# kant2002/GGMLSharp

Hardware: AMD Instinct MI355X
Metric: effective GFLOP/s, Q4_0 mul_mat 4096x4096x4096 (2*M*K*N / step time) (higher is better)
Workload: dtype i8

## Files before the change

### ggmlsharp_amd/csrc/gemm_qmx.hip

```cpp
#include "common.h"
#include "plan.h"
#include <cstdlib>
#include <utility>

#if !defined(GGML_HIP_DEV)
#undef GGML_MX_DBG
#undef GGML_MX_XCD1D
#endif
#ifndef GGML_MX_DBG
#define GGML_MX_DBG 0
#endif
#ifndef GGML_MX_XCD1D
#define GGML_MX_XCD1D 0
#endif

namespace {

using f32x4 = __attribute__((ext_vector_type(4))) float;
using f32x16 = __attribute__((ext_vector_type(16))) float;
using u32x4 = __attribute__((ext_vector_type(4))) uint32_t;
using u32x2 = __attribute__((ext_vector_type(2))) uint32_t;
using i32x8 = __attribute__((ext_vector_type(8))) int;

typedef __attribute__((address_space(3))) void lds_void;
// ... 6 lines not shown
    __builtin_amdgcn_raw_ptr_buffer_load_lds(r, (lds_void *)l, 16, (int)voff, (int)soff, 0, 0);
}

template <typename F, int... Is>
__device__ __forceinline__ void static_for_impl(F &&f, std::integer_sequence<int, Is...>) {
    (f(std::integral_constant<int, Is>{}), ...);
}
template <int N, typename F>
__device__ __forceinline__ void static_for(F &&f) {
    static_for_impl(f, std::make_integer_sequence<int, N>{});
}

#ifdef K3M_CLOCK
__device__ unsigned long long k3m_clock_buf[8192 * 2];
__device__ unsigned int k3m_where_buf[8192 * 2];
#endif

#ifndef GGML_MX_FULLDRAIN
#define GGML_MX_FULLDRAIN 0
#endif
template <int TYPE, int WMT, int WNT, int WGM, int WGN, int KB>
struct Cfg {
    static constexpr int TM = WGM * WMT * 32, TN = WGN * WNT * 32, NT = WGM * WGN * 64;
    static constexpr int A16_BYTES = KB * 2 * TN * 16;
    static constexpr int A8_BYTES = KB * 2 * TN * 8;
    static constexpr int NSC = (TYPE == GGML_TYPE_Q4_1) ? 2 : 1;
    static constexpr int SC_BYTES = KB * TN * 4;
    static constexpr int STAGE = A16_BYTES + A8_BYTES + NSC * SC_BYTES;
    static constexpr int TOTAL = 2 * STAGE;
    static constexpr int P = NT / TN;
    static_assert(NT % TN == 0 && (P == 1 || P == 2 || P == 4), "chunk decomposition");
    static_assert((KB * 2 * TN) % NT == 0 && (KB * TN) % NT == 0, "DMA rounds");
    static constexpr int A16_ROUNDS = KB * 2 * TN / NT, A8_ROUNDS = KB * TN / NT;
    static constexpr int SC_CHUNKS = KB * TN / 4;
    static_assert((SC_CHUNKS % 64 == 0 || SC_CHUNKS == 32) && SC_CHUNKS <= NT, "scale DMA is whole waves (or the first half of one: 32-column tiles)");
    static constexpr int NPIECE = A16_ROUNDS + A8_ROUNDS + 1;
    static constexpr int DRAIN_T = (KB - 1) * WMT * WNT + WMT * WNT / 2;
    static constexpr int PP = (NPIECE + DRAIN_T - 1) / DRAIN_T;
    static_assert(PP <= 3, "at most three DMA pieces per tile");
};

template <int TYPE, int WMT, int WNT, int WGM, int WGN, int KB, int FB, int KSP, int VS>
__global__ __launch_bounds__(WGM * WGN * 64 * KSP, (VS > 1 && WGM * WGN * KSP == 4 && WMT * WNT == 2 ? 3 : 2))
void gemm_qmx_kernel(const uint8_t *__restrict__ w6a, const uint8_t *__restrict__ w6b, const float *__restrict__ wd,
                     const float *__restrict__ wm, const uint8_t *__restrict__ a6, const float *__restrict__ ad,
                     const float *__restrict__ asd, float *__restrict__ dst, int M, int N, int Mpad, int Npad, int nstages,
                     int ldd, int tiles_m, int tiles_n, uint32_t w6a_bytes, uint32_t wd_bytes, uint32_t a_bytes,
                     uint32_t ad_bytes, uint32_t dst_bytes, const mm_epilogue ep) {
    using C = Cfg<TYPE, WMT, WNT, WGM, WGN, KB>;
    constexpr int NTILE = WMT * WNT, P = C::P;
    constexpr int NF = (TYPE == GGML_TYPE_Q4_0 || TYPE == GGML_TYPE_Q4_1) ? 1 : 2;
    static_assert(KB % 2 == 0, "fragment buffers alternate by k-block parity");
    static_assert(VS == 1 || (KSP == 1 && (VS == 2 || VS == 4)) || (KSP == 2 && VS == 2), "virtual split forms");
    constexpr int KV = KSP * VS;
    extern __shared__ __attribute__((aligned(16))) uint8_t smem[];

    const int lane = threadIdx.x & 63;
    const int wave_all = __builtin_amdgcn_readfirstlane(threadIdx.x >> 6);
    const int grp = wave_all / (WGM * WGN);
    const int wave = wave_all % (WGM * WGN);
    const int tid = wave * 64 + lane;
    const int l31 = lane & 31, hh = lane >> 5;
    const int wn = wave / WGM, wm_ = wave % WGM;
    uint8_t *const gsm = smem + grp * C::TOTAL;

    const int nwg = tiles_m * tiles_n;
    const int bid = blockIdx.x, xcd = bid & 7, q8 = nwg >> 3, r8 = nwg & 7;
    int tm_i, tn_i;
// ... 144 lines not shown
                else asm volatile("s_waitcnt vmcnt(0)" ::: "memory");
            }
            if constexpr (t < LAST) issue(std::integral_constant<int, t + 1>{});
            f32x16 &ac = acc[i][j];
            static_for<4>([&](auto gc) {
                constexpr int q = decltype(gc)::value;
                float t0, t1, t2, t3;
                if constexpr (t == 0 && q == 0) asm volatile("s_nop 11" : "+v"(tacc[0]));
                if constexpr (q == 0 && t < LAST && TYPE == GGML_TYPE_Q4_1 && (((t + 1) / NTILE) & 1)) {
                    constexpr int tn = t + 1, j1 = (tn % NTILE) / WMT, i1 = tn % WMT;
                    asm volatile("" : "+v"(acc[i1][j1]));
                }
                if constexpr ((GGML_MX_DBG & 16) != 0) {
                    asm volatile("" : "+v"(ac[4 * q]) : "v"(tacc[t & 1]), "v"(da[q]), "v"(dw), "v"(tacc[(t + 1) & 1]));
                } else if constexpr (q == 0 && t < LAST) {
                    asm volatile("v_mul_f32 %4, %8, %12\n\tv_mul_f32 %5, %9, %13\n\tv_mul_f32 %6, %10, %14\n\tv_mul_f32 %7, %11, %15\n\t"
                                 "v_fmac_f32 %0, %4, %16\n\tv_fmac_f32 %1, %5, %16\n\tv_fmac_f32 %2, %6, %16\n\tv_fmac_f32 %3, %7, %16"
                                 : "+v"(ac[0]), "+v"(ac[1]), "+v"(ac[2]), "+v"(ac[3]), "=&v"(t0), "=&v"(t1), "=&v"(t2), "=&v"(t3)
                                 : "v"(tacc[t & 1][0]), "v"(tacc[t & 1][1]), "v"(tacc[t & 1][2]), "v"(tacc[t & 1][3]), "v"(da[0][0]),
                                   "v"(da[0][1]), "v"(da[0][2]), "v"(da[0][3]), "v"(dw), "v"(tacc[(t + 1) & 1]));
                } else {
                    asm volatile("v_mul_f32 %4, %8, %12\n\tv_mul_f32 %5, %9, %13\n\tv_mul_f32 %6, %10, %14\n\tv_mul_f32 %7, %11, %15\n\t"
                                 "v_fmac_f32 %0, %4, %16\n\tv_fmac_f32 %1, %5, %16\n\tv_fmac_f32 %2, %6, %16\n\tv_fmac_f32 %3, %7, %16"
                                 : "+v"(ac[4 * q + 0]), "+v"(ac[4 * q + 1]), "+v"(ac[4 * q + 2]), "+v"(ac[4 * q + 3]), "=&v"(t0), "=&v"(t1),
                                   "=&v"(t2), "=&v"(t3)
                                 : "v"(tacc[t & 1][4 * q + 0]), "v"(tacc[t & 1][4 * q + 1]), "v"(tacc[t & 1][4 * q + 2]),
                                   "v"(tacc[t & 1][4 * q + 3]), "v"(da[q][0]), "v"(da[q][1]), "v"(da[q][2]), "v"(da[q][3]), "v"(dw));
                }
                if constexpr (i == WMT - 1 && bb * WNT + j + 1 < KB * WNT && !(GGML_MX_DBG & (2 | 32)))
                    fetch_da(std::integral_constant<int, bb * WNT + j + 1>{}, gc);
            });
        });
    };

    static_assert(FB <= KB, "fragment look-ahead stays within two stages");
    const int s_first = grp * VS;
    static_for<C::NPIECE>([&](auto pc) { dma_piece(s_first, 0, pc); });
    static_for<WMT>([&](auto ic) {
// ... 2 lines not shown
    asm volatile("s_waitcnt vmcnt(0) lgkmcnt(0)" ::: "memory");
    __builtin_amdgcn_s_barrier();
    asm volatile("" ::: "memory");
    f32x16 sav[VS > 1 ? WMT : 1][VS > 1 ? WNT : 1];
    const int niter = VS * ((nstages + KV - 1) / KV);
    int sc = s_first, pass = 0;
#ifdef K3M_CLOCK
    const unsigned long long clk_c0 = __builtin_readcyclecounter(), clk_r0 = wall_clock64();
#endif
#ifndef GGML_MX_PRIO
#define GGML_MX_PRIO 15
#endif
#ifndef GGML_MX_PRIO_ON
#define GGML_MX_PRIO_ON 8
#endif
    bool younger = false;
    if constexpr (WGM * WGN * KSP == 4 && GGML_MX_PRIO != 0) {
        uint32_t hwid;
        asm volatile("s_getreg_b32 %0, hwreg(HW_REG_HW_ID)" : "=s"(hwid));
        younger = (hwid & 1u) != 0 && nwg <= 512;
    }
    for (int it = 0; it < niter; ++it) {
        if constexpr (WGM * WGN * KSP == 4 && GGML_MX_PRIO != 0) {
            if (younger) { if (it % GGML_MX_PRIO < GGML_MX_PRIO_ON) __builtin_amdgcn_s_setprio(1); else __builtin_amdgcn_s_setprio(0); }
        }
        int sn = sc + KV, pn = pass;
        if (VS > 1 && sn >= nstages) { pn = pass + 1; sn = pn < VS ? grp * VS + pn : nstages; }
        if ((KSP == 1 && VS == 1) || sc < nstages) compute(sc, sn, it);
        if constexpr (KSP == 1 && VS == 1 && !GGML_MX_FULLDRAIN) asm volatile("s_waitcnt lgkmcnt(0)" ::: "memory");
        else asm volatile("s_waitcnt vmcnt(0) lgkmcnt(0)" ::: "memory");
        if (!(GGML_MX_DBG & 1)) __builtin_amdgcn_s_barrier();
        asm volatile("" ::: "memory");
        if constexpr (VS > 1) {
            if (pn != pass && pn < VS) {
#pragma unroll
                for (int i = 0; i < WMT; ++i)
#pragma unroll
                    for (int j = 0; j < WNT; ++j) {
                        sav[i][j] = pass == 0 ? acc[i][j] : sav[i][j] + acc[i][j];
#pragma unroll
                        for (int r = 0; r < 16; ++r) acc[i][j][r] = 0.0f;
                    }
            }
        }
        sc = sn; pass = pn;
    }
#ifdef K3M_CLOCK
    {
        asm volatile("" : "+v"(acc[0][0]));
        const unsigned long long c1 = __builtin_readcyclecounter(), r1 = wall_clock64();
        const size_t slot = (size_t)blockIdx.x * (WGM * WGN * KSP) + wave_all;
        if (lane == 0 && slot < 8192) { k3m_clock_buf[2 * slot] = c1 - clk_c0; k3m_clock_buf[2 * slot + 1] = r1 - clk_r0; }
        uint32_t hw, xcc;
        asm volatile("s_getreg_b32 %0, hwreg(HW_REG_HW_ID)\n\ts_getreg_b32 %1, hwreg(HW_REG_XCC_ID)" : "=s"(hw), "=s"(xcc));
        if (lane == 0 && slot < 8192) { k3m_where_buf[2 * slot] = hw; k3m_where_buf[2 * slot + 1] = xcc; }
    }
#endif

    if constexpr (KSP > 1) {
        constexpr int GRP_FLOATS = WGM * WGN * NTILE * 16 * 64;
        static_assert((KSP - 1) * VS * GRP_FLOATS * 4 <= KSP * C::TOTAL, "K-split exchange fits the stage buffers");
        float *xch = (float *)smem + (size_t)wave * (NTILE * 16 * 64) + lane;
        if (grp != 0) {
#pragma unroll
            for (int i = 0; i < WMT; ++i)
#pragma unroll
                for (int j = 0; j < WNT; ++j)
#pragma unroll
                    for (int r = 0; r < 16; ++r) {
                        if constexpr (VS > 1) xch[(size_t)((grp - 1) * VS) * GRP_FLOATS + ((i * WNT + j) * 16 + r) * 64] = sav[i][j][r];
                        xch[(size_t)((grp - 1) * VS + VS - 1) * GRP_FLOATS + ((i * WNT + j) * 16 + r) * 64] = acc[i][j][r];
// ... 13 lines not shown
        const float *xch = (const float *)smem + (size_t)wave * (NTILE * 16 * 64) + lane;
#pragma unroll
        for (int g = VS; g < KV; ++g)
#pragma unroll
            for (int i = 0; i < WMT; ++i)
#pragma unroll
                for (int j = 0; j < WNT; ++j)
#pragma unroll
                    for (int r = 0; r < 16; ++r) acc[i][j][r] += xch[(size_t)(g - VS) * GRP_FLOATS + ((i * WNT + j) * 16 + r) * 64];
    }

    (void)dst_bytes;
    const rsrc_t rD = make_rsrc(dst + (size_t)n0 * ldd + m0, 0xFFFFFFFFu);
    const bool full = n0 + C::TN <= N && m0 + C::TM <= M;
    const uint32_t lane_off = (uint32_t)((4 * hh * ldd + l31) * 4);
    if (ep.mode == 3) {
        rsrc_t rP[MM_PUSH_MAX];
#pragma unroll
        for (int k = 0; k < MM_PUSH_MAX; ++k) rP[k] = make_rsrc((k < ep.npush ? ep.push[k] : dst) + (size_t)n0 * ldd + m0, 0xFFFFFFFFu);
#pragma unroll
        for (int i = 0; i < WMT; ++i)
#pragma unroll
            for (int j = 0; j < WNT; ++j) {
                const int mb = (wm_ * WMT + i) * 32, nb = (wn * WNT + j) * 32;
                if (m0 + mb >= M || n0 + nb >= N) continue;
                const bool mok = m0 + mb + l31 < M;
#pragma unroll
                for (int r = 0; r < 16; ++r) {
                    const int nr = nb + (r & 3) + 8 * (r >> 2);
                    const float v = acc[i][j][r];
                    if (!(mok && n0 + nr + 4 * hh < N)) continue;
                    const uint32_t so = (uint32_t)(nr * ldd + mb) * 4u, vb = __builtin_bit_cast(uint32_t, v);
                    __builtin_amdgcn_raw_buffer_store_b32(vb, rD, (int)lane_off, (int)so, 0);
#pragma unroll
                    for (int k = 0; k < MM_PUSH_MAX; ++k)
                        if (k < ep.npush) __builtin_amdgcn_raw_buffer_store_b32(vb, rP[k], (int)lane_off, (int)so, 0);
                }
            }
        return;
    }
    if (ep.mode != 0) {
        const int lda = (int)ep.ld_add, ld2 = (int)ep.ld2;
        const rsrc_t rS = make_rsrc(ep.mode == 1 ? ep.addend + (size_t)n0 * lda + m0 : dst, 0xFFFFFFFFu);
        const rsrc_t rD2 = make_rsrc(ep.mode == 1 ? ep.dst2 + (size_t)n0 * ld2 + m0 : dst, 0xFFFFFFFFu);
        const uint32_t lane_s = (uint32_t)((4 * hh * lda + l31) * 4), lane_2 = (uint32_t)((4 * hh * ld2 + l31) * 4);
#pragma unroll
        for (int i = 0; i < WMT; ++i)
#pragma unroll
            for (int j = 0; j < WNT; ++j) {
                const int mb = (wm_ * WMT + i) * 32, nb = (wn * WNT + j) * 32;
                if (m0 + mb >= M || n0 + nb >= N) continue;
                const bool mok = m0 + mb + l31 < M;
#pragma unroll
                for (int r = 0; r < 16; ++r) {
                    const int nr = nb + (r & 3) + 8 * (r >> 2);
                    const float v = acc[i][j][r];
                    if (!(mok && n0 + nr + 4 * hh < N)) continue;
                    if (ep.mode == 2) {
                        const float o = v * ep.scale;
                        __builtin_amdgcn_raw_buffer_store_b32(__builtin_bit_cast(uint32_t, o), rD, (int)lane_off, (int)((uint32_t)(nr * ldd + mb) * 4u), 0);
                    } else {
                        __builtin_amdgcn_raw_buffer_store_b32(__builtin_bit_cast(uint32_t, v), rD, (int)lane_off, (int)((uint32_t)(nr * ldd + mb) * 4u), 0);
                        const float a = __builtin_bit_cast(float, __builtin_amdgcn_raw_buffer_load_b32(rS, (int)lane_s, (int)((uint32_t)(nr * lda + mb) * 4u), 0));
                        const float o = v + a;
                        __builtin_amdgcn_raw_buffer_store_b32(__builtin_bit_cast(uint32_t, o), rD2, (int)lane_2, (int)((uint32_t)(nr * ld2 + mb) * 4u), 0);
                    }
                }
            }
        return;
    }
    if (full) {
#pragma unroll
        for (int i = 0; i < WMT; ++i)
#pragma unroll
            for (int j = 0; j < WNT; ++j)
#pragma unroll
                for (int r = 0; r < 16; ++r) {
                    const int nr = (wn * WNT + j) * 32 + (r & 3) + 8 * (r >> 2), mb = (wm_ * WMT + i) * 32;
                    const float v = acc[i][j][r];
                    __builtin_amdgcn_raw_buffer_store_b32(__builtin_bit_cast(uint32_t, v), rD, (int)lane_off,
                                                          (int)((uint32_t)(nr * ldd + mb) * 4u), 0);
                }
    } else {
#pragma unroll
        for (int i = 0; i < WMT; ++i)
#pragma unroll
            for (int j = 0; j < WNT; ++j) {
                const int mb = (wm_ * WMT + i) * 32, nb = (wn * WNT + j) * 32;
                if (m0 + mb >= M || n0 + nb >= N) continue;
                const bool mok = m0 + mb + l31 < M;
#pragma unroll
                for (int r = 0; r < 16; ++r) {
                    const int nr = nb + (r & 3) + 8 * (r >> 2);
                    const float v = acc[i][j][r];
                    if (mok && n0 + nr + 4 * hh < N)
                        __builtin_amdgcn_raw_buffer_store_b32(__builtin_bit_cast(uint32_t, v), rD, (int)lane_off,
                                                              (int)((uint32_t)(nr * ldd + mb) * 4u), 0);
                }
            }
    }
}

#ifdef K3S_TRACE
__device__ unsigned long long k3s_trace_buf[2048 * 2 * 8];
#define K3S_STAMP(k) do { if (lane == 0 && (wave == 0 || wave == KS - 1) && blockIdx.x < 2048) \
        k3s_trace_buf[((size_t)blockIdx.x * 2 + (wave != 0)) * 8 + (k)] = wall_clock64(); } while (0)
#else
#define K3S_STAMP(k) do { } while (0)
#endif
template <int TYPE, int KS, int NP, bool ROT, int WMT>
__device__ __forceinline__
void gemm_qmx_small_body(const uint8_t *__restrict__ w6a, const uint8_t *__restrict__ w6b, const float *__restrict__ wd,
                         const float *__restrict__ wm, const uint8_t *__restrict__ a6, const float *__restrict__ ad,
                         const float *__restrict__ asd, float *__restrict__ dst, int M, int N, int Mpad, int Npad, int nbkp,
                         int nloc, int ldd, uint32_t w6a_bytes, uint32_t wd_bytes, uint32_t a_bytes, uint32_t ad_bytes,
// ... 405 lines not shown
};
template <int TYPE, int KS, int NP, bool ROT, int WMT>
__global__ __launch_bounds__(KS * 64, 1)
void gemm_qmx_small_multi_kernel(const mxs_set ws, const uint8_t *__restrict__ a6, const float *__restrict__ ad, const float *__restrict__ asd,
                                 int N, int Npad, int nbkp, int nloc, uint32_t a_bytes, uint32_t ad_bytes, int ncol) {
    const int b = (int)blockIdx.x;
    const int k = (b >= ws.wg_end[0]) + (b >= ws.wg_end[1]) + (b >= ws.wg_end[2]);
    const int first = k == 0 ? 0 : k == 1 ? ws.wg_end[0] : k == 2 ? ws.wg_end[1] : ws.wg_end[2];
#define MXS(f) (k == 0 ? ws.f[0] : k == 1 ? ws.f[1] : k == 2 ? ws.f[2] : ws.f[3])
    const mm_epilogue ep{0, nullptr, 0, nullptr, 0, 1.0f};
    gemm_qmx_small_body<TYPE, KS, NP, ROT, WMT>(MXS(a), MXS(b), MXS(d), MXS(m), a6, ad, asd, MXS(dst), MXS(M), N, MXS(Mpad), Npad, nbkp, nloc, MXS(ldd),
                                                MXS(wa_bytes), MXS(wd_bytes), a_bytes, ad_bytes, ep, b - first, ((k == 0 ? ws.wg_end[0] : k == 1 ? ws.wg_end[1] : k == 2 ? ws.wg_end[2] : ws.wg_end[3]) - first) / ncol);
#undef MXS
}

template <int TYPE, int WMT, int WNT, int WGM, int WGN, int KB, int FB, int KSP = 1, int VS = 1>
hipError_t launch_cfg(const ggml_hip_weight *w, act_planes p, int64_t N, float *dst, int64_t ldd, hipStream_t st, const mm_epilogue *ep) {
    using C = Cfg<TYPE, WMT, WNT, WGM, WGN, KB>;
    if (w->Mpad % C::TM != 0 || p.Npad % C::TN != 0 || !w->q6a || !w->q6b) return hipErrorInvalidValue;
    const int tiles_m = (int)((w->M + C::TM - 1) / C::TM), tiles_n = (int)((N + C::TN - 1) / C::TN);
    const int nstages = (int)((w->nbk + KB - 1) / KB);
    static_assert(K_STAGE_PAD % KB == 0, "stage padding");
    const uint64_t nba = (uint64_t)pad_kblocks(w->nbk);
    constexpr int NF = (TYPE == GGML_TYPE_Q4_0 || TYPE == GGML_TYPE_Q4_1) ? 1 : 2;
    const uint64_t wq_bytes = (nba + K_LOOKAHEAD) * (uint64_t)w->Mpad * 16 * NF;
    const uint64_t wd_bytes = (nba + K_LOOKAHEAD) * (uint64_t)w->Mpad * 4, a_bytes = nba * 48 * (uint64_t)p.Npad;
    const uint64_t ad_bytes = nba * (uint64_t)p.Npad * 4, dst_bytes = ((uint64_t)(N - 1) * (uint64_t)ldd + (uint64_t)w->M) * 4;
    constexpr uint64_t LIM = 0xFFFFFFFFull;
    if (wq_bytes > LIM || a_bytes > LIM || (uint64_t)C::TN * (uint64_t)ldd * 4 > LIM) return hipErrorNotSupported;
    return launch_lds(kfn<gemm_qmx_kernel<TYPE, WMT, WNT, WGM, WGN, KB, FB, KSP, VS>>, dim3((unsigned)(tiles_m * tiles_n)), C::NT * KSP, C::TOTAL * KSP,
                      C::TOTAL * KSP, st, w->q6a, w->q6b, w->d, w->m, (const uint8_t *)p.a8, p.ad, (const float *)p.as, dst, (int)w->M, (int)N, (int)w->Mpad,
                      (int)p.Npad, nstages, (int)ldd, tiles_m, tiles_n, (uint32_t)wq_bytes, (uint32_t)wd_bytes, (uint32_t)a_bytes, (uint32_t)ad_bytes,
                      (uint32_t)dst_bytes, epilogue_or_none(ep));
}

template <int TYPE>
hipError_t launch_small(const ggml_hip_weight *w, const mm_plan &pl, act_planes p, int64_t N, float *dst, int64_t ldd, hipStream_t st, const mm_epilogue *ep) {
    constexpr int KS = 8;
    constexpr bool Q40 = TYPE == GGML_TYPE_Q4_0, Q41 = TYPE == GGML_TYPE_Q4_1;
    if (!w->q6a || !w->q6b) return hipErrorInvalidValue;
    const int nbkp = (int)pad_kblocks(w->nbk);
    const int nloc = pl.nloc, wmt = pl.wmt;
    const uint64_t nba = (uint64_t)nbkp;
    const uint64_t wq_bytes = (nba + K_LOOKAHEAD) * (uint64_t)w->Mpad * 16, wd_bytes = (nba + K_LOOKAHEAD) * (uint64_t)w->Mpad * 4;
    const uint64_t a_bytes = nba * 48 * (uint64_t)p.Npad, ad_bytes = nba * (uint64_t)p.Npad * 4;
// ... 85 lines not shown
}

#ifndef MX_SMALL_FB
#define MX_SMALL_FB 2
#endif
template <int TYPE>
hipError_t launch_typed(const ggml_hip_weight *w, const mm_plan &pl, act_planes p, int64_t N, float *dst, int64_t ldd, hipStream_t st, const mm_epilogue *ep) {
    constexpr bool Q40 = TYPE == GGML_TYPE_Q4_0, Q4 = Q40 || TYPE == GGML_TYPE_Q4_1;
    if (pl.family == MMF_K3S_MX) {
        if constexpr (Q4) return launch_small<TYPE>(w, pl, p, N, dst, ldd, st, ep);
        return hipErrorInvalidValue;
    }
    if (pl.family == MMF_K3P_MX) return launch_gemm_qmx_mid(w, pl, p, N, dst, ldd, st, ep);
    if (pl.family != MMF_MX) return hipErrorInvalidValue;
    switch (pl.form) {
    case MXF_256x128:     if constexpr (Q40) return launch_cfg<TYPE, 2, 4, 4, 1, 4, 2>(w, p, N, dst, ldd, st, ep); break;
    case MXF_N32_H64:     return launch_cfg<TYPE, 1, 1, 2, 1, 4, 2, 4>(w, p, N, dst, ldd, st, ep);
    case MXF_N32_H32:     return launch_cfg<TYPE, 1, 1, 1, 1, 4, 2, 4>(w, p, N, dst, ldd, st, ep);
    case MXF_S4_H128:     if constexpr (Q40) return launch_cfg<TYPE, 1, 2, 4, 1, 4, MX_SMALL_FB, 4>(w, p, N, dst, ldd, st, ep); break;
    case MXF_S4_H64:      return launch_cfg<TYPE, 1, 2, 2, 1, 4, MX_SMALL_FB, 4>(w, p, N, dst, ldd, st, ep);
    case MXF_S4_H32:      return launch_cfg<TYPE, 1, 2, 1, 1, 4, MX_SMALL_FB, 4>(w, p, N, dst, ldd, st, ep);
    case MXF_S2V2_H64:    if constexpr (Q40) return launch_cfg<TYPE, 1, 2, 2, 1, 4, 2, 2, 2>(w, p, N, dst, ldd, st, ep); break;
    case MXF_S2_H128:     return launch_cfg<TYPE, 1, 2, 4, 1, 4, 2, 2>(w, p, N, dst, ldd, st, ep);
    case MXF_S2_H64:      return launch_cfg<TYPE, 1, 2, 2, 1, 4, 2, 2>(w, p, N, dst, ldd, st, ep);
    case MXF_128x128:     return launch_cfg<TYPE, 2, 2, 2, 2, 4, 2>(w, p, N, dst, ldd, st, ep);
    case MXF_64x64:       if constexpr (Q40) return launch_cfg<TYPE, 1, 1, 2, 2, 4, 2>(w, p, N, dst, ldd, st, ep); break;
    case MXF_128x64:      return launch_cfg<TYPE, 1, 2, 4, 1, 4, 2>(w, p, N, dst, ldd, st, ep);
    default: break;
    }
    return hipErrorInvalidValue;
}
// ... 29 lines not shown
```

### ggmlsharp_amd/csrc/plan.cpp

```cpp
#include "common.h"
#include "plan.h"

namespace {

thread_local int t_force_gemm = 0;

inline bool is_quant(int t) { return t >= GGML_TYPE_Q4_0 && t <= GGML_TYPE_Q8_1; }
inline bool min_type(int t) { return t == GGML_TYPE_Q4_1 || t == GGML_TYPE_Q5_1; }
inline int64_t cdiv(int64_t a, int64_t b) { return (a + b - 1) / b; }
constexpr uint64_t LIM32 = 0xFFFFFFFFull;

int64_t gemv_rows_max(int t) { return t == GGML_TYPE_Q4_2 ? GEMV_WIDE_MAX_N : GEMV_MAX_N; }

constexpr int KS8 = 8;
int k3p_mx_nloc(int64_t K) { int n = (int)cdiv(pad_kblocks(K / QK), KS8); return n + (n & 1); }
int k3p_i8_nloc(int64_t K) { int n = (int)cdiv(pad_kblocks(K / QK), KS8); return n + (n & 1); }
bool k3p_lds_ok(int nloc) { return nloc <= K3P_MAX_SLICES * K3P_SLICE_ROWS; }

constexpr int64_t K3_DUAL_MIN = 33, K3_DUAL_MAX = 512;
constexpr int64_t K3S_KMIN = 32;
int64_t k3_dual_wgs(int64_t K) { return K >= 11008 ? 192 : 160; }
int64_t q41_pair_min(int64_t K) { return K >= 11008 ? 129 : 65; }
bool q8_small_serves(int type, int64_t K, int64_t N, bool i8_only = false, bool kq = false) {
    if (K / QK < K3S_KMIN || K / QK > 1024 || plan_force_gemm() != 0) return false;
// ... 7 lines not shown
    if (K / QK < 64 || !k3p_lds_ok(k3p_i8_nloc(K)) || plan_force_gemm() != 0) return false;
    const bool dual = K / QK <= 1024;
    const int64_t nmin = !dual ? 129 : type == GGML_TYPE_Q4_1 ? q41_pair_min(K) : K3_DUAL_MIN;
    if (type == GGML_TYPE_Q4_2) return N >= nmin;
    const int64_t top = type == GGML_TYPE_Q4_1 ? 1024 : type == GGML_TYPE_Q5_1 ? INT64_MAX : 3072;
    return (type == GGML_TYPE_Q8_0 || type == GGML_TYPE_Q5_0 || type == GGML_TYPE_Q5_1 || type == GGML_TYPE_Q4_1) && N >= nmin && N <= top;
}

int f16_image_kind(int type) { return type == GGML_TYPE_Q8_0 ? 2 : 1; }

int k3_i8_arith(int type) { return 300 + (min_type(type) ? 1 : 0) + (type == GGML_TYPE_Q8_0 ? 2 : 0) + (type == GGML_TYPE_Q4_2 ? 4 : 0); }

}

int plan_force_gemm() { return t_force_gemm; }
void plan_set_force_gemm(int which) { t_force_gemm = which < 0 || which > 3 ? 0 : which; }

int plan_image_kind(int type, int64_t K, int64_t N) {
    const int force = plan_force_gemm();
    if (q8_mid_serves(type, K, N)) return min_type(type) ? ACT_IMAGE_MIN_PIECES : 0;
    if (q8_small_serves(type, K, N)) return min_type(type) ? ACT_IMAGE_MIN_PIECES : 0;
    if (N <= 4 || force == 1) return 0;
    if (N <= GEMV_MAX_N && !(force == 0 && (type == GGML_TYPE_Q4_0 || type == GGML_TYPE_Q4_1) && K / QK >= K3S_KMIN)) return 0;
    if (type == GGML_TYPE_Q4_2) return 0;
    const uint64_t nba = (uint64_t)pad_kblocks(K / QK);
    if (nba * 64 * (uint64_t)pad_act(N) > LIM32) return 0;
    if (force == 2) return f16_image_kind(type);
    if (type == GGML_TYPE_Q5_1 && force == 3) return 0;
    if (force == 3 || type == GGML_TYPE_Q4_0 || type == GGML_TYPE_Q4_1) return 3;
    return ((N <= 512 || N >= 1024) && K / QK >= 8) ? f16_image_kind(type) : 0;
}
// ... 102 lines not shown
    p.ksplit = g.ksp * g.vs; p.kstyle = p.ksplit > 1 ? MMK_STAGE_SETS : MMK_CHAIN; p.kunit = 4;
    p.wgs = cdiv(M, p.tile_m) * cdiv(N, p.tile_n);
}

void plan_mx(mm_plan &p, int type, int64_t M, int64_t Mpad, int64_t K, int64_t N) {
    const int64_t nbk = K / QK;
    const int64_t tm256 = cdiv(M, 256), tm128 = cdiv(M, 128), tn128 = cdiv(N, 128), t64 = cdiv(M, 64) * cdiv(N, 64);
    const bool q40 = type == GGML_TYPE_Q4_0, q4 = q40 || type == GGML_TYPE_Q4_1;
    static const FormGeo geo[] = {{2, 4, 4, 1, 1, 1}, {}, {1, 1, 2, 1, 4, 1}, {1, 1, 1, 1, 4, 1}, {1, 2, 4, 1, 4, 1}, {1, 2, 2, 1, 4, 1},
                                  {1, 2, 1, 1, 4, 1}, {1, 2, 2, 1, 2, 2}, {1, 2, 4, 1, 2, 1}, {1, 2, 2, 1, 2, 1}, {2, 2, 2, 2, 1, 1}, {1, 1, 2, 2, 1, 1}, {1, 2, 4, 1, 1, 1}};
    auto take = [&](int f) {
        p.family = MMF_MX; p.image = 3; p.form = f;
        set_staged_geo(p, geo[f], M, N);
        p.arith = 400 + (type == GGML_TYPE_Q4_1 ? 1 + (p.tiles_per_wave == 1 ? 1 : 0) : type == GGML_TYPE_Q4_0 ? 0 : 10 + type);
        p.flags |= MM_FLAG_EPILOGUE_FUSED;
    };
    if (q40 && tm256 * tn128 >= 257 && N > 512) return take(MXF_256x128);
    if (q40 && N >= K3_DUAL_MIN && N <= K3_DUAL_MAX && nbk >= 64) {
        if (t64 >= k3_dual_wgs(K) && plan_k3p_mx(p, M, Mpad, K, N)) return;
        if (plan_k3s_mx(p, type, M, Mpad, K, N)) return;
        if (plan_k3p_mx(p, M, Mpad, K, N)) return;
    }
    if (N <= (q40 ? 128 : 256) && nbk >= 16) {
        if (q4) {
            const int ncmax = nbk < 64 ? 2 : (K >= 11008 || !q40) ? 4 : 2;
            if (N <= 32 * ncmax && nbk >= K3S_KMIN && plan_k3s_mx(p, type, M, Mpad, K, N)) return;
        }
        if (N <= 32) return take(t64 < 160 ? MXF_N32_H32 : MXF_N32_H64);
        if (t64 < 160) return take(MXF_S4_H32);
        return take(t64 <= 320 || !q40 ? MXF_S4_H64 : MXF_S4_H128);
// ... 209 lines not shown
```

### ggmlsharp_amd/csrc/plan.h

```cpp
#pragma once
#include <stdint.h>

enum mm_family {
    MMF_NONE = 0,
    MMF_GEMV_FUSED = 1,
    MMF_GEMV_ROWS = 2,
    MMF_K3S_MX = 3,
    MMF_K3S_I8 = 4,
    MMF_K3P_MX = 5,
    MMF_K3P_I8 = 6,
    MMF_MX = 7,
    MMF_F16 = 8,
    MMF_I8 = 9,
    MMF_DENSE = 10,
    MMF_DENSE_GEMV = 11,
    MMF_DENSE16 = 12,
    MMF_DENSE32 = 13,
};

enum mm_kstyle { MMK_CHAIN = 0, MMK_STAGE_SETS = 1, MMK_RANGES = 2, MMK_WORKERS = 3 };

enum { MM_FLAG_WIDE = 1, MM_FLAG_EPILOGUE_FUSED = 2, MM_FLAG_PERSISTENT = 4, MM_FLAG_Q8K = 8, MM_FLAG_NEEDS_WORK = 16,
       MM_FLAG_MIN_PIECES = 32 ,
       MM_FLAG_MIN_PASS = 64  };

enum mx_form {
    MXF_256x128 = 0,
    MXF_N32_H64 = 2,
    MXF_N32_H32,
    MXF_S4_H128,
    MXF_S4_H64,
    MXF_S4_H32,
    MXF_S2V2_H64,
    MXF_S2_H128,
    MXF_S2_H64,
    MXF_128x128,
    MXF_64x64,
    MXF_128x64,
};
// ... 16 lines not shown
    int waves;
    int tiles_per_wave;
    int64_t wgs;
    int flags;
    int nloc, wmt;
};

mm_plan plan_mul_mat(int type, int ext_type, int64_t M, int64_t K, int64_t N, bool one_call = true);
uint32_t plan_tree_id(const mm_plan &p);
mm_plan plan_mul_mat_group(int type, int ext_type, const int64_t *M, const int64_t *Mpad, int n, int64_t K, int64_t N);
struct k3s_slots { int slots; bool rot; int rows; int lds; };
k3s_slots plan_k3s_slots(const mm_plan &p, int type);
int plan_image_kind(int type, int64_t K, int64_t N);
int plan_force_gemm();
void plan_set_force_gemm(int which);
```

### include/ggml_hip_ext.h

```cpp
#ifndef GGML_HIP_EXT_H
#define GGML_HIP_EXT_H

#include "ggml_hip.h"

#ifdef __cplusplus
extern "C" {
#endif
#if defined(__GNUC__)
#pragma GCC visibility push(default)
#endif

#define GGML_HIP_TYPE_Q5_K 113
#define GGML_HIP_TYPE_Q4_K 112
#define GGML_HIP_TYPE_Q6_K 114
#define GGML_HIP_TYPE_Q3_K 111
#define GGML_HIP_TYPE_Q2_K 110
#define GGML_HIP_TYPE_IQ4_NL 120
#define GGML_HIP_TYPE_IQ4_XS 123
#define GGML_HIP_TYPE_BF16 130


int  ggml_hip_graph_outputs(const void *const *host_ptrs, int n);
int  ggml_hip_graph_begin_keyed(uint64_t key);
void ggml_hip_debug_scope_counters(uint64_t *observed, uint64_t *captured, uint64_t *replayed, uint64_t *refused);
// ... 2 lines not shown
void ggml_hip_debug_weight_cache_stats(uint64_t *entries, uint64_t *bytes, uint64_t *evictions);


int    ggml_hip_act_image_kind(int type, int64_t K, int64_t N);
enum {
    GGML_HIP_MMF_GEMV_FUSED = 1, GGML_HIP_MMF_GEMV_ROWS = 2, GGML_HIP_MMF_K3S_MX = 3, GGML_HIP_MMF_K3S_I8 = 4, GGML_HIP_MMF_K3P_MX = 5,
    GGML_HIP_MMF_K3P_I8 = 6, GGML_HIP_MMF_MX = 7, GGML_HIP_MMF_F16 = 8, GGML_HIP_MMF_I8 = 9, GGML_HIP_MMF_DENSE = 10,
    GGML_HIP_MMF_DENSE_GEMV = 11, GGML_HIP_MMF_DENSE16 = 12, GGML_HIP_MMF_DENSE32 = 13
};
enum {
    GGML_HIP_PLAN_WIDE = 1,
    GGML_HIP_PLAN_EPILOGUE_FUSED = 2,
    GGML_HIP_PLAN_PERSISTENT = 4, GGML_HIP_PLAN_Q8K = 8,
    GGML_HIP_PLAN_NEEDS_WORK = 16,
    GGML_HIP_PLAN_MIN_PIECES = 32,
    GGML_HIP_PLAN_MIN_PASS = 64
};
typedef struct ggml_hip_mm_plan_t {
    int32_t  family, image_kind, form;
    uint32_t tree_id;
    int32_t  arith, ksplit, kstyle, kunit;
    int32_t  tile_m, tile_n, waves, tiles_per_wave;
    int64_t  workgroups;
    int32_t  flags;
} ggml_hip_mm_plan_t;
int    ggml_hip_mm_plan(int type, int64_t M, int64_t K, int64_t N, ggml_hip_mm_plan_t *out);
void   ggml_hip_debug_force_gemm(int which);
int    ggml_hip_debug_q2k_min_pass_dev(const ggml_hip_weight *w, int64_t N, float *d_dst, int64_t ldd, const void *d_work, size_t work_bytes,
                                       int form, void *stream);
int    ggml_hip_quantize_act_dev(const float *d_src1, int64_t N, int64_t K, int64_t ld1, void *d_work, size_t work_bytes,
                                 int image_kind, void *stream);
// ... 86 lines not shown
```

Baseline: 851,500.

## Reorder last K-stage tile-major so output stores overlap remaining MFMA work

Adds a TAIL variant of the 256x128 Q4_0 MX kernel. Full-tile workgroups skip the last pipelined stage and run it in tile-major order, loading weight fragments directly from global memory and storing each output tile as soon as its K accumulation finishes. The aim is to overlap the epilogue stores with the remaining MFMA work instead of leaving them as a serial tail. The planner enables it when the grid has at most 512 workgroups and there are at least four k-units. The cost is extra direct global weight loads in the tail, more register pressure and code size, and a debug flag bit to turn the path off.

```diff
diff --git a/ggmlsharp_amd/csrc/gemm_qmx.hip b/ggmlsharp_amd/csrc/gemm_qmx.hip
--- a/ggmlsharp_amd/csrc/gemm_qmx.hip
+++ b/ggmlsharp_amd/csrc/gemm_qmx.hip
@@ -44,11 +44,14 @@
 #ifdef K3M_CLOCK
 __device__ unsigned long long k3m_clock_buf[8192 * 2];
 __device__ unsigned int k3m_where_buf[8192 * 2];
+__device__ unsigned int k3m_store_buf[8192 * 4];
 #endif
 
 #ifndef GGML_MX_FULLDRAIN
 #define GGML_MX_FULLDRAIN 0
 #endif
+#define K3M_SACC_ASM "v_mul_f32 %4, %8, %12\n\tv_mul_f32 %5, %9, %13\n\tv_mul_f32 %6, %10, %14\n\tv_mul_f32 %7, %11, %15\n\t" \
+                     "v_fmac_f32 %0, %4, %16\n\tv_fmac_f32 %1, %5, %16\n\tv_fmac_f32 %2, %6, %16\n\tv_fmac_f32 %3, %7, %16"
 template <int TYPE, int WMT, int WNT, int WGM, int WGN, int KB>
 struct Cfg {
     static constexpr int TM = WGM * WMT * 32, TN = WGN * WNT * 32, NT = WGM * WGN * 64;
@@ -70,7 +73,7 @@
     static_assert(PP <= 3, "at most three DMA pieces per tile");
 };
 
-template <int TYPE, int WMT, int WNT, int WGM, int WGN, int KB, int FB, int KSP, int VS>
+template <int TYPE, int WMT, int WNT, int WGM, int WGN, int KB, int FB, int KSP, int VS, bool TAIL = false>
 __global__ __launch_bounds__(WGM * WGN * 64 * KSP, (VS > 1 && WGM * WGN * KSP == 4 && WMT * WNT == 2 ? 3 : 2))
 void gemm_qmx_kernel(const uint8_t *__restrict__ w6a, const uint8_t *__restrict__ w6b, const float *__restrict__ wd,
                      const float *__restrict__ wm, const uint8_t *__restrict__ a6, const float *__restrict__ ad,
@@ -82,6 +85,7 @@
     constexpr int NF = (TYPE == GGML_TYPE_Q4_0 || TYPE == GGML_TYPE_Q4_1) ? 1 : 2;
     static_assert(KB % 2 == 0, "fragment buffers alternate by k-block parity");
     static_assert(VS == 1 || (KSP == 1 && (VS == 2 || VS == 4)) || (KSP == 2 && VS == 2), "virtual split forms");
+    static_assert(!TAIL || (KSP == 1 && VS == 1 && NF == 1 && TYPE != GGML_TYPE_Q4_1 && 2 * WNT >= KB && FB == 2), "tile-major last stage: the unsplit one-digit forms");
     constexpr int KV = KSP * VS;
     extern __shared__ __attribute__((aligned(16))) uint8_t smem[];
 
@@ -256,14 +260,12 @@
                 if constexpr ((GGML_MX_DBG & 16) != 0) {
                     asm volatile("" : "+v"(ac[4 * q]) : "v"(tacc[t & 1]), "v"(da[q]), "v"(dw), "v"(tacc[(t + 1) & 1]));
                 } else if constexpr (q == 0 && t < LAST) {
-                    asm volatile("v_mul_f32 %4, %8, %12\n\tv_mul_f32 %5, %9, %13\n\tv_mul_f32 %6, %10, %14\n\tv_mul_f32 %7, %11, %15\n\t"
-                                 "v_fmac_f32 %0, %4, %16\n\tv_fmac_f32 %1, %5, %16\n\tv_fmac_f32 %2, %6, %16\n\tv_fmac_f32 %3, %7, %16"
+                    asm volatile(K3M_SACC_ASM
                                  : "+v"(ac[0]), "+v"(ac[1]), "+v"(ac[2]), "+v"(ac[3]), "=&v"(t0), "=&v"(t1), "=&v"(t2), "=&v"(t3)
                                  : "v"(tacc[t & 1][0]), "v"(tacc[t & 1][1]), "v"(tacc[t & 1][2]), "v"(tacc[t & 1][3]), "v"(da[0][0]),
                                    "v"(da[0][1]), "v"(da[0][2]), "v"(da[0][3]), "v"(dw), "v"(tacc[(t + 1) & 1]));
                 } else {
-                    asm volatile("v_mul_f32 %4, %8, %12\n\tv_mul_f32 %5, %9, %13\n\tv_mul_f32 %6, %10, %14\n\tv_mul_f32 %7, %11, %15\n\t"
-                                 "v_fmac_f32 %0, %4, %16\n\tv_fmac_f32 %1, %5, %16\n\tv_fmac_f32 %2, %6, %16\n\tv_fmac_f32 %3, %7, %16"
+                    asm volatile(K3M_SACC_ASM
                                  : "+v"(ac[4 * q + 0]), "+v"(ac[4 * q + 1]), "+v"(ac[4 * q + 2]), "+v"(ac[4 * q + 3]), "=&v"(t0), "=&v"(t1),
                                    "=&v"(t2), "=&v"(t3)
                                  : "v"(tacc[t & 1][4 * q + 0]), "v"(tacc[t & 1][4 * q + 1]), "v"(tacc[t & 1][4 * q + 2]),
@@ -296,6 +298,7 @@
 #ifndef GGML_MX_PRIO_ON
 #define GGML_MX_PRIO_ON 8
 #endif
+    const bool tail_wg = TAIL && ep.mode == 0 && n0 + C::TN <= N && m0 + C::TM <= M;
     bool younger = false;
     if constexpr (WGM * WGN * KSP == 4 && GGML_MX_PRIO != 0) {
         uint32_t hwid;
@@ -308,6 +311,7 @@
         }
         int sn = sc + KV, pn = pass;
         if (VS > 1 && sn >= nstages) { pn = pass + 1; sn = pn < VS ? grp * VS + pn : nstages; }
+        if constexpr (TAIL) { if (it == niter - 1 && tail_wg) break; }
         if ((KSP == 1 && VS == 1) || sc < nstages) compute(sc, sn, it);
         if constexpr (KSP == 1 && VS == 1 && !GGML_MX_FULLDRAIN) asm volatile("s_waitcnt lgkmcnt(0)" ::: "memory");
         else asm volatile("s_waitcnt vmcnt(0) lgkmcnt(0)" ::: "memory");
@@ -328,15 +332,22 @@
         sc = sn; pass = pn;
     }
 #ifdef K3M_CLOCK
-    {
-        asm volatile("" : "+v"(acc[0][0]));
+    const size_t clk_slot = (size_t)blockIdx.x * (WGM * WGN * KSP) + wave_all;
+    auto clk_loop_end = [&] {
+        asm volatile("" : "+v"(acc[WMT - 1][WNT - 1]));
         const unsigned long long c1 = __builtin_readcyclecounter(), r1 = wall_clock64();
-        const size_t slot = (size_t)blockIdx.x * (WGM * WGN * KSP) + wave_all;
-        if (lane == 0 && slot < 8192) { k3m_clock_buf[2 * slot] = c1 - clk_c0; k3m_clock_buf[2 * slot + 1] = r1 - clk_r0; }
+        if (lane == 0 && clk_slot < 8192) { k3m_clock_buf[2 * clk_slot] = c1 - clk_c0; k3m_clock_buf[2 * clk_slot + 1] = r1 - clk_r0; }
         uint32_t hw, xcc;
         asm volatile("s_getreg_b32 %0, hwreg(HW_REG_HW_ID)\n\ts_getreg_b32 %1, hwreg(HW_REG_XCC_ID)" : "=s"(hw), "=s"(xcc));
-        if (lane == 0 && slot < 8192) { k3m_where_buf[2 * slot] = hw; k3m_where_buf[2 * slot + 1] = xcc; }
-    }
+        if (lane == 0 && clk_slot < 8192) { k3m_where_buf[2 * clk_slot] = hw; k3m_where_buf[2 * clk_slot + 1] = xcc; }
+    };
+    auto clk_stamp = [&](int k) {
+        asm volatile("" ::: "memory");
+        const unsigned long long r1 = wall_clock64();
+        if (lane == 0 && clk_slot < 8192) k3m_store_buf[4 * clk_slot + k] = (unsigned int)(r1 - clk_r0);
+    };
+    clk_stamp(0);
+    if (!tail_wg) clk_loop_end();
 #endif
 
     if constexpr (KSP > 1) {
@@ -380,91 +391,163 @@
     const rsrc_t rD = make_rsrc(dst + (size_t)n0 * ldd + m0, 0xFFFFFFFFu);
     const bool full = n0 + C::TN <= N && m0 + C::TM <= M;
     const uint32_t lane_off = (uint32_t)((4 * hh * ldd + l31) * 4);
-    if (ep.mode == 3) {
-        rsrc_t rP[MM_PUSH_MAX];
-#pragma unroll
-        for (int k = 0; k < MM_PUSH_MAX; ++k) rP[k] = make_rsrc((k < ep.npush ? ep.push[k] : dst) + (size_t)n0 * ldd + m0, 0xFFFFFFFFu);
-#pragma unroll
-        for (int i = 0; i < WMT; ++i)
-#pragma unroll
-            for (int j = 0; j < WNT; ++j) {
-                const int mb = (wm_ * WMT + i) * 32, nb = (wn * WNT + j) * 32;
-                if (m0 + mb >= M || n0 + nb >= N) continue;
-                const bool mok = m0 + mb + l31 < M;
-#pragma unroll
-                for (int r = 0; r < 16; ++r) {
-                    const int nr = nb + (r & 3) + 8 * (r >> 2);
-                    const float v = acc[i][j][r];
-                    if (!(mok && n0 + nr + 4 * hh < N)) continue;
-                    const uint32_t so = (uint32_t)(nr * ldd + mb) * 4u, vb = __builtin_bit_cast(uint32_t, v);
+    auto store_tile = [&](auto ic, auto jc, auto kc) {
+        constexpr int i = decltype(ic)::value, j = decltype(jc)::value, kind = decltype(kc)::value;
+        const int mb = (wm_ * WMT + i) * 32, nb = (wn * WNT + j) * 32;
+        if constexpr (kind == 0) {
+#pragma unroll
+            for (int r = 0; r < 16; ++r) {
+                const int nr = nb + (r & 3) + 8 * (r >> 2);
+                const float v = acc[i][j][r];
+                __builtin_amdgcn_raw_buffer_store_b32(__builtin_bit_cast(uint32_t, v), rD, (int)lane_off, (int)((uint32_t)(nr * ldd + mb) * 4u), 0);
+            }
+        } else {
+            if (m0 + mb >= M || n0 + nb >= N) return;
+            const bool mok = m0 + mb + l31 < M;
+            const int lda = (int)ep.ld_add, ld2 = (int)ep.ld2;
+            rsrc_t rS = rD, rD2 = rD, rP[MM_PUSH_MAX];
+            uint32_t lane_s = 0, lane_2 = 0;
+            if constexpr (kind == 2) {
+                rS = make_rsrc(ep.mode == 1 ? ep.addend + (size_t)n0 * lda + m0 : dst, 0xFFFFFFFFu);
+                rD2 = make_rsrc(ep.mode == 1 ? ep.dst2 + (size_t)n0 * ld2 + m0 : dst, 0xFFFFFFFFu);
+                lane_s = (uint32_t)((4 * hh * lda + l31) * 4), lane_2 = (uint32_t)((4 * hh * ld2 + l31) * 4);
+            }
+            if constexpr (kind == 3) {
+#pragma unroll
+                for (int k = 0; k < MM_PUSH_MAX; ++k) rP[k] = make_rsrc((k < ep.npush ? ep.push[k] : dst) + (size_t)n0 * ldd + m0, 0xFFFFFFFFu);
+            }
+#pragma unroll
+            for (int r = 0; r < 16; ++r) {
+                const int nr = nb + (r & 3) + 8 * (r >> 2);
+                const float v = acc[i][j][r];
+                if (!(mok && n0 + nr + 4 * hh < N)) continue;
+                const uint32_t so = (uint32_t)(nr * ldd + mb) * 4u, vb = __builtin_bit_cast(uint32_t, v);
+                if constexpr (kind == 1) {
+                    __builtin_amdgcn_raw_buffer_store_b32(vb, rD, (int)lane_off, (int)so, 0);
+                } else if constexpr (kind == 3) {
                     __builtin_amdgcn_raw_buffer_store_b32(vb, rD, (int)lane_off, (int)so, 0);
 #pragma unroll
                     for (int k = 0; k < MM_PUSH_MAX; ++k)
                         if (k < ep.npush) __builtin_amdgcn_raw_buffer_store_b32(vb, rP[k], (int)lane_off, (int)so, 0);
+                } else if (ep.mode == 2) {
+                    const float o = v * ep.scale;
+                    __builtin_amdgcn_raw_buffer_store_b32(__builtin_bit_cast(uint32_t, o), rD, (int)lane_off, (int)so, 0);
+                } else {
+                    __builtin_amdgcn_raw_buffer_store_b32(vb, rD, (int)lane_off, (int)so, 0);
+                    const float a = __builtin_bit_cast(float, __builtin_amdgcn_raw_buffer_load_b32(rS, (int)lane_s, (int)((uint32_t)(nr * lda + mb) * 4u), 0));
+                    const float o = v + a;
+                    __builtin_amdgcn_raw_buffer_store_b32(__builtin_bit_cast(uint32_t, o), rD2, (int)lane_2, (int)((uint32_t)(nr * ld2 + mb) * 4u), 0);
                 }
             }
+        }
+    };
+    using K0 = std::integral_constant<int, 0>;
+    using K1 = std::integral_constant<int, 1>;
+    using K2 = std::integral_constant<int, 2>;
+    using K3 = std::integral_constant<int, 3>;
+
+    if constexpr (TAIL) {
+        if (tail_wg) {
+        const int s_last = sc, kb0 = s_last * KB;
+        const uint8_t *sp = gsm + ((niter - 1) & 1) * C::STAGE;
+        const uint8_t *sA16 = sp + ((size_t)(hh * C::TN + wn * WNT * 32 + l31)) * 16;
+        const uint8_t *sA8 = sp + C::A16_BYTES + ((size_t)(hh * C::TN + wn * WNT * 32 + l31)) * 8;
+        const float *sDa = (const float *)(sp + C::A16_BYTES + C::A8_BYTES) + wn * WNT * 32 + 4 * hh;
+        struct WF { u32x4 lo; u32x2 hi; float d; };
+        WF wf[WMT][KB];
+        auto load_wf = [&](auto ic, auto bc) {
+            constexpr int i = decltype(ic)::value, bb = decltype(bc)::value;
+            wf[i][bb].lo = __builtin_amdgcn_raw_buffer_load_b128(rWa, (int)(offA + 512u * i), (int)((uint32_t)(kb0 + bb) * wa_blk), 0);
+            wf[i][bb].hi = __builtin_amdgcn_raw_buffer_load_b64(rWb, (int)(offB + 256u * i), (int)((uint32_t)(kb0 + bb) * wb_blk), 0);
+            wf[i][bb].d = __builtin_bit_cast(float, __builtin_amdgcn_raw_buffer_load_b32(rWd, (int)(offD + 128u * i), (int)((uint32_t)(kb0 + bb) * d_blk), 0));
+        };
+        static_for<KB>([&](auto bc) {
+            constexpr int bb = decltype(bc)::value;
+            if constexpr (bb < FB) { wf[0][bb].lo = frag[bb].lo[0][0]; wf[0][bb].hi = frag[bb].hi[0][0]; wf[0][bb].d = frag[bb].d[0]; }
+            else load_wf(std::integral_constant<int, 0>{}, bc);
+        });
+        constexpr int NSTEP = NTILE * KB, LASTU = NSTEP - 1;
+        u32x4 af_lo;
+        u32x2 af_hi;
+        f32x4 da[4];
+        f32x16 tacc[2];
+        const f32x16 zero = {0, 0, 0, 0, 0, 0, 0, 0, 0, 0, 0, 0, 0, 0, 0, 0};
+        auto fetch_af = [&](auto uc) {
+            constexpr int u = decltype(uc)::value, bb = u % KB, j = (u / KB) % WNT;
+            af_lo = *(const u32x4 *)(sA16 + (bb * 2 * C::TN + 32 * j) * 16);
+            af_hi = *(const u32x2 *)(sA8 + (bb * 2 * C::TN + 32 * j) * 8);
+        };
+        auto fetch_da = [&](auto uc, auto gc) {
+            constexpr int u = decltype(uc)::value, bb = u % KB, j = (u / KB) % WNT, q = decltype(gc)::value;
+            da[q] = *(const f32x4 *)(sDa + bb * C::TN + 32 * j + 8 * q);
+        };
+        auto issue = [&](auto uc) {
+            constexpr int u = decltype(uc)::value, bb = u % KB, i = u / (KB * WNT);
+            const WF &f = wf[i][bb];
+            const i32x8 a = {(int)af_lo[0], (int)af_lo[1], (int)af_lo[2], (int)af_lo[3], (int)af_hi[0], (int)af_hi[1], 0, 0};
+            const i32x8 b = {(int)f.lo[0], (int)f.lo[1], (int)f.lo[2], (int)f.lo[3], (int)f.hi[0], (int)f.hi[1], 0, 0};
+            tacc[u & 1] = __builtin_amdgcn_mfma_scale_f32_32x32x64_f8f6f4(a, b, zero, 3, 3, 0, scale_a, 0, 127);
+            if constexpr (u < LASTU) fetch_af(std::integral_constant<int, u + 1>{});
+        };
+        fetch_af(std::integral_constant<int, 0>{});
+        static_for<4>([&](auto gc) { fetch_da(std::integral_constant<int, 0>{}, gc); });
+        issue(std::integral_constant<int, 0>{});
+        static_for<NSTEP>([&](auto uc) {
+            constexpr int u = decltype(uc)::value, bb = u % KB, j = (u / KB) % WNT, i = u / (KB * WNT);
+            const float dw = wf[i][bb].d;
+            if constexpr (u < LASTU) issue(std::integral_constant<int, u + 1>{});
+            f32x16 &ac = acc[i][j];
+            static_for<4>([&](auto gc) {
+                constexpr int q = decltype(gc)::value;
+                float t0, t1, t2, t3;
+                if constexpr (u == 0 && q == 0) asm volatile("s_nop 11" : "+v"(tacc[0]));
+                if constexpr (q == 0 && u < LASTU) {
+                    asm volatile(K3M_SACC_ASM
+                                 : "+v"(ac[0]), "+v"(ac[1]), "+v"(ac[2]), "+v"(ac[3]), "=&v"(t0), "=&v"(t1), "=&v"(t2), "=&v"(t3)
+                                 : "v"(tacc[u & 1][0]), "v"(tacc[u & 1][1]), "v"(tacc[u & 1][2]), "v"(tacc[u & 1][3]), "v"(da[0][0]),
+                                   "v"(da[0][1]), "v"(da[0][2]), "v"(da[0][3]), "v"(dw), "v"(tacc[(u + 1) & 1]));
+                } else {
+                    asm volatile(K3M_SACC_ASM
+                                 : "+v"(ac[4 * q + 0]), "+v"(ac[4 * q + 1]), "+v"(ac[4 * q + 2]), "+v"(ac[4 * q + 3]), "=&v"(t0), "=&v"(t1),
+                                   "=&v"(t2), "=&v"(t3)
+                                 : "v"(tacc[u & 1][4 * q + 0]), "v"(tacc[u & 1][4 * q + 1]), "v"(tacc[u & 1][4 * q + 2]),
+                                   "v"(tacc[u & 1][4 * q + 3]), "v"(da[q][0]), "v"(da[q][1]), "v"(da[q][2]), "v"(da[q][3]), "v"(dw));
+                }
+                if constexpr (u < LASTU) fetch_da(std::integral_constant<int, u + 1>{}, gc);
+            });
+            if constexpr (bb == KB - 1) {
+#ifdef K3M_CLOCK
+                if constexpr (u == LASTU) clk_loop_end();
+#endif
+                store_tile(std::integral_constant<int, i>{}, std::integral_constant<int, j>{}, K0{});
+#ifdef K3M_CLOCK
+                if constexpr (u == KB - 1) clk_stamp(1);
+                if constexpr (u == LASTU) clk_stamp(2);
+#endif
+                if constexpr (i + 1 < WMT && 2 * j < KB) {
+                    load_wf(std::integral_constant<int, i + 1>{}, std::integral_constant<int, 2 * j>{});
+                    if constexpr (2 * j + 1 < KB) load_wf(std::integral_constant<int, i + 1>{}, std::integral_constant<int, 2 * j + 1>{});
+                }
+            }
+        });
         return;
-    }
-    if (ep.mode != 0) {
-        const int lda = (int)ep.ld_add, ld2 = (int)ep.ld2;
-        const rsrc_t rS = make_rsrc(ep.mode == 1 ? ep.addend + (size_t)n0 * lda + m0 : dst, 0xFFFFFFFFu);
-        const rsrc_t rD2 = make_rsrc(ep.mode == 1 ? ep.dst2 + (size_t)n0 * ld2 + m0 : dst, 0xFFFFFFFFu);
-        const uint32_t lane_s = (uint32_t)((4 * hh * lda + l31) * 4), lane_2 = (uint32_t)((4 * hh * ld2 + l31) * 4);
-#pragma unroll
-        for (int i = 0; i < WMT; ++i)
-#pragma unroll
-            for (int j = 0; j < WNT; ++j) {
-                const int mb = (wm_ * WMT + i) * 32, nb = (wn * WNT + j) * 32;
-                if (m0 + mb >= M || n0 + nb >= N) continue;
-                const bool mok = m0 + mb + l31 < M;
-#pragma unroll
-                for (int r = 0; r < 16; ++r) {
-                    const int nr = nb + (r & 3) + 8 * (r >> 2);
-                    const float v = acc[i][j][r];
-                    if (!(mok && n0 + nr + 4 * hh < N)) continue;
-                    if (ep.mode == 2) {
-                        const float o = v * ep.scale;
-                        __builtin_amdgcn_raw_buffer_store_b32(__builtin_bit_cast(uint32_t, o), rD, (int)lane_off, (int)((uint32_t)(nr * ldd + mb) * 4u), 0);
-                    } else {
-                        __builtin_amdgcn_raw_buffer_store_b32(__builtin_bit_cast(uint32_t, v), rD, (int)lane_off, (int)((uint32_t)(nr * ldd + mb) * 4u), 0);
-                        const float a = __builtin_bit_cast(float, __builtin_amdgcn_raw_buffer_load_b32(rS, (int)lane_s, (int)((uint32_t)(nr * lda + mb) * 4u), 0));
-                        const float o = v + a;
-                        __builtin_amdgcn_raw_buffer_store_b32(__builtin_bit_cast(uint32_t, o), rD2, (int)lane_2, (int)((uint32_t)(nr * ld2 + mb) * 4u), 0);
-                    }
-                }
-            }
-        return;
-    }
-    if (full) {
-#pragma unroll
-        for (int i = 0; i < WMT; ++i)
-#pragma unroll
-            for (int j = 0; j < WNT; ++j)
-#pragma unroll
-                for (int r = 0; r < 16; ++r) {
-                    const int nr = (wn * WNT + j) * 32 + (r & 3) + 8 * (r >> 2), mb = (wm_ * WMT + i) * 32;
-                    const float v = acc[i][j][r];
-                    __builtin_amdgcn_raw_buffer_store_b32(__builtin_bit_cast(uint32_t, v), rD, (int)lane_off,
-                                                          (int)((uint32_t)(nr * ldd + mb) * 4u), 0);
-                }
-    } else {
-#pragma unroll
-        for (int i = 0; i < WMT; ++i)
-#pragma unroll
-            for (int j = 0; j < WNT; ++j) {
-                const int mb = (wm_ * WMT + i) * 32, nb = (wn * WNT + j) * 32;
-                if (m0 + mb >= M || n0 + nb >= N) continue;
-                const bool mok = m0 + mb + l31 < M;
-#pragma unroll
-                for (int r = 0; r < 16; ++r) {
-                    const int nr = nb + (r & 3) + 8 * (r >> 2);
-                    const float v = acc[i][j][r];
-                    if (mok && n0 + nr + 4 * hh < N)
-                        __builtin_amdgcn_raw_buffer_store_b32(__builtin_bit_cast(uint32_t, v), rD, (int)lane_off,
-                                                              (int)((uint32_t)(nr * ldd + mb) * 4u), 0);
-                }
-            }
-    }
+        }
+    }
+
+    auto store_all = [&](auto kc) {
+        static_for<NTILE>([&](auto tc) {
+            constexpr int t = decltype(tc)::value;
+            store_tile(std::integral_constant<int, t / WNT>{}, std::integral_constant<int, t % WNT>{}, kc);
+#ifdef K3M_CLOCK
+            if constexpr (t == 0) clk_stamp(1);
+            if constexpr (t == NTILE - 1) clk_stamp(2);
+#endif
+        });
+    };
+    if (ep.mode == 3) store_all(K3{});
+    else if (ep.mode != 0) store_all(K2{});
+    else if (full) store_all(K0{});
+    else store_all(K1{});
 }
 
 #ifdef K3S_TRACE
@@ -900,7 +983,7 @@
 #undef MXS
 }
 
-template <int TYPE, int WMT, int WNT, int WGM, int WGN, int KB, int FB, int KSP = 1, int VS = 1>
+template <int TYPE, int WMT, int WNT, int WGM, int WGN, int KB, int FB, int KSP = 1, int VS = 1, bool TAIL = false>
 hipError_t launch_cfg(const ggml_hip_weight *w, act_planes p, int64_t N, float *dst, int64_t ldd, hipStream_t st, const mm_epilogue *ep) {
     using C = Cfg<TYPE, WMT, WNT, WGM, WGN, KB>;
     if (w->Mpad % C::TM != 0 || p.Npad % C::TN != 0 || !w->q6a || !w->q6b) return hipErrorInvalidValue;
@@ -914,7 +997,7 @@
     const uint64_t ad_bytes = nba * (uint64_t)p.Npad * 4, dst_bytes = ((uint64_t)(N - 1) * (uint64_t)ldd + (uint64_t)w->M) * 4;
     constexpr uint64_t LIM = 0xFFFFFFFFull;
     if (wq_bytes > LIM || a_bytes > LIM || (uint64_t)C::TN * (uint64_t)ldd * 4 > LIM) return hipErrorNotSupported;
-    return launch_lds(kfn<gemm_qmx_kernel<TYPE, WMT, WNT, WGM, WGN, KB, FB, KSP, VS>>, dim3((unsigned)(tiles_m * tiles_n)), C::NT * KSP, C::TOTAL * KSP,
+    return launch_lds(kfn<gemm_qmx_kernel<TYPE, WMT, WNT, WGM, WGN, KB, FB, KSP, VS, TAIL>>, dim3((unsigned)(tiles_m * tiles_n)), C::NT * KSP, C::TOTAL * KSP,
                       C::TOTAL * KSP, st, w->q6a, w->q6b, w->d, w->m, (const uint8_t *)p.a8, p.ad, (const float *)p.as, dst, (int)w->M, (int)N, (int)w->Mpad,
                       (int)p.Npad, nstages, (int)ldd, tiles_m, tiles_n, (uint32_t)wq_bytes, (uint32_t)wd_bytes, (uint32_t)a_bytes, (uint32_t)ad_bytes,
                       (uint32_t)dst_bytes, epilogue_or_none(ep));
@@ -1030,7 +1113,10 @@
     if (pl.family == MMF_K3P_MX) return launch_gemm_qmx_mid(w, pl, p, N, dst, ldd, st, ep);
     if (pl.family != MMF_MX) return hipErrorInvalidValue;
     switch (pl.form) {
-    case MXF_256x128:     if constexpr (Q40) return launch_cfg<TYPE, 2, 4, 4, 1, 4, 2>(w, p, N, dst, ldd, st, ep); break;
+    case MXF_256x128:
+        if constexpr (Q40) return (pl.flags & MM_FLAG_TILE_TAIL) ? launch_cfg<TYPE, 2, 4, 4, 1, 4, 2, 1, 1, true>(w, p, N, dst, ldd, st, ep)
+                                                                 : launch_cfg<TYPE, 2, 4, 4, 1, 4, 2>(w, p, N, dst, ldd, st, ep);
+        break;
     case MXF_N32_H64:     return launch_cfg<TYPE, 1, 1, 2, 1, 4, 2, 4>(w, p, N, dst, ldd, st, ep);
     case MXF_N32_H32:     return launch_cfg<TYPE, 1, 1, 1, 1, 4, 2, 4>(w, p, N, dst, ldd, st, ep);
     case MXF_S4_H128:     if constexpr (Q40) return launch_cfg<TYPE, 1, 2, 4, 1, 4, MX_SMALL_FB, 4>(w, p, N, dst, ldd, st, ep); break;
diff --git a/ggmlsharp_amd/csrc/plan.cpp b/ggmlsharp_amd/csrc/plan.cpp
--- a/ggmlsharp_amd/csrc/plan.cpp
+++ b/ggmlsharp_amd/csrc/plan.cpp
@@ -3,6 +3,7 @@
 
 namespace {
 
+thread_local bool t_no_tile_tail = false;
 thread_local int t_force_gemm = 0;
 
 inline bool is_quant(int t) { return t >= GGML_TYPE_Q4_0 && t <= GGML_TYPE_Q8_1; }
@@ -45,7 +46,12 @@
 }
 
 int plan_force_gemm() { return t_force_gemm; }
-void plan_set_force_gemm(int which) { t_force_gemm = which < 0 || which > 3 ? 0 : which; }
+void plan_set_force_gemm(int which) {
+    t_no_tile_tail = which >= 0 && (which & 16) != 0;
+    if (which >= 0) which &= ~16;
+    t_force_gemm = which < 0 || which > 3 ? 0 : which;
+}
+bool plan_no_tile_tail() { return t_no_tile_tail; }
 
 int plan_image_kind(int type, int64_t K, int64_t N) {
     const int force = plan_force_gemm();
@@ -178,6 +184,7 @@
         set_staged_geo(p, geo[f], M, N);
         p.arith = 400 + (type == GGML_TYPE_Q4_1 ? 1 + (p.tiles_per_wave == 1 ? 1 : 0) : type == GGML_TYPE_Q4_0 ? 0 : 10 + type);
         p.flags |= MM_FLAG_EPILOGUE_FUSED;
+        if (f == MXF_256x128 && p.wgs <= 512 && cdiv(nbk, (int64_t)p.kunit) >= 4 && !plan_no_tile_tail()) p.flags |= MM_FLAG_TILE_TAIL;
     };
     if (q40 && tm256 * tn128 >= 257 && N > 512) return take(MXF_256x128);
     if (q40 && N >= K3_DUAL_MIN && N <= K3_DUAL_MAX && nbk >= 64) {
diff --git a/ggmlsharp_amd/csrc/plan.h b/ggmlsharp_amd/csrc/plan.h
--- a/ggmlsharp_amd/csrc/plan.h
+++ b/ggmlsharp_amd/csrc/plan.h
@@ -22,7 +22,8 @@
 
 enum { MM_FLAG_WIDE = 1, MM_FLAG_EPILOGUE_FUSED = 2, MM_FLAG_PERSISTENT = 4, MM_FLAG_Q8K = 8, MM_FLAG_NEEDS_WORK = 16,
        MM_FLAG_MIN_PIECES = 32 ,
-       MM_FLAG_MIN_PASS = 64  };
+       MM_FLAG_MIN_PASS = 64 ,
+       MM_FLAG_TILE_TAIL = 128  };
 
 enum mx_form {
     MXF_256x128 = 0,
@@ -69,3 +70,4 @@
 int plan_image_kind(int type, int64_t K, int64_t N);
 int plan_force_gemm();
 void plan_set_force_gemm(int which);
+bool plan_no_tile_tail();
diff --git a/include/ggml_hip_ext.h b/include/ggml_hip_ext.h
--- a/include/ggml_hip_ext.h
+++ b/include/ggml_hip_ext.h
@@ -40,7 +40,8 @@
     GGML_HIP_PLAN_PERSISTENT = 4, GGML_HIP_PLAN_Q8K = 8,
     GGML_HIP_PLAN_NEEDS_WORK = 16,
     GGML_HIP_PLAN_MIN_PIECES = 32,
-    GGML_HIP_PLAN_MIN_PASS = 64
+    GGML_HIP_PLAN_MIN_PASS = 64,
+    GGML_HIP_PLAN_TILE_TAIL = 128
 };
 typedef struct ggml_hip_mm_plan_t {
     int32_t  family, image_kind, form;
```

Measured after the change: 851,000, median of 2. Within noise of the previous version (-0.1%).
